# mkkellogg/GaussianSplats3D

Measured on AMD Instinct MI355X. Metric: Msplats/s sorted+rasterized at 1920x1080 SH-2, higher is better.
Workload: dtype int32 keys / f32 raster; 1 GPU; C3: garden.ply stand-in, SH2, 1920x1080; splats=5800000, sh_degree=2, width=1920, height=1080, cull=off (R=N), sort_precision_bits=16, streams=one (SURVEY.md 8d: sort -> draw on a single stream), parallelism=1 GPU, sort=full list (R = N)

## Files before the change

### gaussiansplats3d_amd/csrc/extreme_set.cpp

```cpp
#include "extreme_set.hpp"

#include <math.h>

#include <algorithm>
#include <new>
#include <utility>

namespace {

typedef __int128 i128;

struct P { int32_t x, y, z; };
inline bool operator==(const P& a, const P& b) { return a.x == b.x && a.y == b.y && a.z == b.z; }
inline bool lex_less(const P& a, const P& b) { return a.x != b.x ? a.x < b.x : (a.y != b.y ? a.y < b.y : a.z < b.z); }
struct D3 { int64_t x, y, z; };
inline D3 sub(const P& a, const P& b) { return {(int64_t)a.x - b.x, (int64_t)a.y - b.y, (int64_t)a.z - b.z}; }
struct N3 { i128 x, y, z; };
inline N3 cross(const D3& u, const D3& v) {
    return {(i128)u.y * v.z - (i128)u.z * v.y, (i128)u.z * v.x - (i128)u.x * v.z, (i128)u.x * v.y - (i128)u.y * v.x};
}
inline i128 dot(const N3& n, const D3& d) { return n.x * d.x + n.y * d.y + n.z * d.z; }
inline bool is_zero(const N3& n) { return n.x == 0 && n.y == 0 && n.z == 0; }
inline double len2(const N3& n) { return (double)n.x * (double)n.x + (double)n.y * (double)n.y + (double)n.z * (double)n.z; }
inline double dabs128(i128 v) { return fabs((double)v); }
// ... 266 lines not shown
        } else {
            if (h.vert.size() > cap || flt.work > budget) break;
            if (round >= 1 && now > (size_t)64 * cap && now * 10 > prev * 7) break;
            if (round >= 2 && now * 100 > prev * 97) break;
        }
        prev = now;
        size_t joined = 0;
        for (size_t f = 0; f < flt.best.size(); f++)
            if (flt.best[f] > 0 && h.insert(flt.best_p[f])) joined++;
        if (!joined) break;
    }
    if (s.size() > cap) return false;
    dedupe(s);
    out.swap(s);
    return true;
}

}

bool gs_extreme_set(const int32_t* a, size_t na, const int32_t* b, size_t nb, uint32_t cap, std::vector<int32_t>& out) {
    out.clear();
    try {
        std::vector<P> s;
        const Src src = {a, na, b, nb};
        if (!build(src, cap, s)) return false;
        emit(s, out);
        return true;
    } catch (const std::bad_alloc&) {
        out.clear();
        return false;
    }
}

extern "C" int gs_debug_extreme_set(const int32_t* prior_aos4, uint32_t prior_count, const int32_t* aos4, uint32_t count, uint32_t cap,
                                    int32_t* out_aos4, uint32_t* out_count) {
    if (!out_aos4 || !out_count || (prior_count && !prior_aos4) || (count && !aos4)) return -1;
    *out_count = 0;
    std::vector<int32_t> out;
    if (!gs_extreme_set(prior_aos4, prior_count, aos4, count, cap, out)) return 1;
    std::copy(out.begin(), out.end(), out_aos4);
    *out_count = (uint32_t)(out.size() / 4);
    return 0;
}
```

### gaussiansplats3d_amd/csrc/extreme_set.hpp

```cpp
#pragma once
#include <cstddef>
#include <cstdint>
#include <vector>

constexpr uint32_t GS_EXTREME_CAP = 4096;

bool gs_extreme_set(const int32_t* a, size_t na, const int32_t* b, size_t nb, uint32_t cap, std::vector<int32_t>& out);

extern "C" int gs_debug_extreme_set(const int32_t* prior_aos4, uint32_t prior_count, const int32_t* aos4, uint32_t count, uint32_t cap,
                                    int32_t* out_aos4, uint32_t* out_count);
```

### gaussiansplats3d_amd/csrc/gs_internal.hpp

```cpp
#pragma once
#include <hip/hip_runtime.h>
#include <stdint.h>
#include <stdio.h>
#include <stdlib.h>
#include <string.h>
#include <new>
#include <utility>
#include <vector>

#include "../../include/gsplat_hip.h"
#include "draw_plan.hpp"

void gs_set_error(const char* fmt, ...);

#define GS_HIP(expr)                                                                              \
    do {                                                                                          \
        hipError_t _e = (expr);                                                                   \
        if (_e != hipSuccess) {                                                                   \
            gs_set_error("%s failed: %s (%s:%d)", #expr, hipGetErrorString(_e), __FILE__, __LINE__); \
            return GS_ERR_HIP;                                                                    \
        }                                                                                         \
    } while (0)

#define GS_REQUIRE(cond, msg)                                    \
// ... 210 lines not shown
    gs_mesh* result_mesh = nullptr;
    const uint32_t* result_unmap = nullptr;
    uint32_t result_payload_max = 0;
    uint32_t gathered = 0;
    bool has_gathered = false;
    bool gathered_on_device = false;
    DevBuf gathered_dev;
    gs_tree* pending_tree = nullptr;
    bool pending_keep_zeroed = false;
    uint32_t centers_version = 0;
    DevBuf pay_in;
    DevBuf leaf_centers, leaf_pos;
    uint64_t leaf_cache_tree = 0;
    uint32_t leaf_cache_centers = 0, leaf_cache_layout = 0, leaf_cache_uploaded = 0;
    const void* leaf_cache_mesh = nullptr;
    uint32_t last_render = 0, last_sort = 0, last_passes = 0;
    bool last_identity = true;
    bool has_result = false;
    bool frustum_cull = false;
    bool visibility_cull = false;
    bool last_culled = false;
    const SortFrame* result_frame = nullptr;
    DevBuf keep_mask;
    DevBuf chunk_counts;
    DevBuf mask_copy;
    bool last_vis_culled = false;
    bool dev_distances = false;
    uint32_t dev_distances_count = 0;
    bool dev_distances_integer = false;
    hipEvent_t ev_handover = nullptr;
    std::vector<int32_t> extreme;
    bool extreme_ok = true;
    uint32_t extreme_version = 0;
    uint32_t clean_slot = 3;
    bool last_known_range = false;
    int32_t last_range_lo = 0, last_range_hi = 0;
    uint32_t last_pass0_slot = 0;
    bool last_narrow = false;
    bool keys_stale = false;
    int32_t stale_im[3] = {0, 0, 0};
    uint32_t stale_count = 0;
};

struct __attribute__((aligned(32))) SplatRec {
    float cx, cy, ax, ay;
    float bx, by;
    uint32_t c0, c1;
};
static_assert(sizeof(SplatRec) == 32, "SplatRec must be one 32-byte sector");

struct RenderFrame {
    uint32_t visible;
    uint32_t entries_lo;
    uint32_t entries_hi;
    uint32_t overflow;
    uint32_t entry_count;
    uint32_t tiles16_lo;
    uint32_t tiles16_hi;
    uint32_t pad;
};

struct ProjectParams {
    float view[16];
    float proj[16];
    float cam_pos[3];
    float focal_x, focal_y;
    float width, height;
    float splat_scale, kernel2d, max_splat_px, inv_focal_adj;
    uint32_t sh_degree;
    uint32_t sh_stored;
    uint32_t cov_half;
// ... 173 lines not shown
```

### gaussiansplats3d_amd/csrc/sorter.hip

```cpp
#include <math.h>
#include <stdlib.h>

#include "extreme_set.hpp"
#include "radix.hpp"

__host__ __device__ static inline int32_t trunc_f64_i32(double v) {
    if (!(v > -2147483649.0 && v < 2147483648.0)) return INT32_MIN;
    return (int32_t)v;
}

constexpr uint32_t MODE_INT = 1, MODE_DYNAMIC = 2, MODE_PRECOMPUTED = 4;
#ifndef GS_KEY_GRID_MULT
#define GS_KEY_GRID_MULT 2
#endif

struct SceneRows {
    int32_t im[GS_MAX_SCENES][4];
    float fm[GS_MAX_SCENES][4];
};

struct KeyParams {
    const uint32_t *cx, *cy, *cz, *cw;
    const uint4* aos;
    const uint32_t* scene_idx;
// ... 2 lines not shown
    const SceneRows* rows;
    int32_t* keys_out;
    SortFrame* frame;
    SortFrame* next_frame;
    uint32_t* digit_total;
    uint32_t sort_start, render_count, mode;
    uint32_t last_splat;
    int32_t im0, im1, im2;
    float fm0, fm1, fm2;
    float mvp[16];
    unsigned long long* keep;
    const uint32_t* count_dev;
    uint32_t ext_minmax;
};

__global__ __launch_bounds__(256) void k_store_scene_rows(SceneRows rows, SceneRows* __restrict__ dst) {
    const uint32_t t = threadIdx.x;
    if (t < GS_MAX_SCENES * 4) {
        dst->im[t >> 2][t & 3] = rows.im[t >> 2][t & 3];
        dst->fm[t >> 2][t & 3] = rows.fm[t >> 2][t & 3];
    }
}

__global__ __launch_bounds__(256) void k_aos4_to_soa(const uint4* __restrict__ aos, uint32_t count, uint32_t from,
                                                     uint32_t* __restrict__ x, uint32_t* __restrict__ y,
                                                     uint32_t* __restrict__ z, uint32_t* __restrict__ w) {
    for (uint32_t i = blockIdx.x * blockDim.x + threadIdx.x; i < count; i += gridDim.x * blockDim.x) {
        const uint4 v = aos[i];
        x[from + i] = v.x;
        y[from + i] = v.y;
        z[from + i] = v.z;
        if (w) w[from + i] = v.w;
    }
}

__device__ __forceinline__ int32_t static_key_int(const KeyParams& p, uint32_t x, uint32_t y, uint32_t z) {
    return (int32_t)(x * (uint32_t)p.im0 + y * (uint32_t)p.im1 + z * (uint32_t)p.im2);
}
__device__ __forceinline__ int32_t static_key_float(const KeyParams& p, uint32_t xb, uint32_t yb, uint32_t zb) {
    float s = __fmul_rn(p.fm0, __uint_as_float(xb));
    s = __fadd_rn(s, __fmul_rn(p.fm1, __uint_as_float(yb)));
    s = __fadd_rn(s, __fmul_rn(p.fm2, __uint_as_float(zb)));
    return trunc_f64_i32((double)s * 4096.0);
}
__device__ __forceinline__ int32_t static_key(const KeyParams& p, uint32_t x, uint32_t y, uint32_t z) {
    return (p.mode & MODE_INT) ? static_key_int(p, x, y, z) : static_key_float(p, x, y, z);
}
__device__ __forceinline__ int32_t static_key_planes(const KeyParams& p, uint32_t i) {
    if (p.mode & MODE_INT) return static_key_int(p, p.cx[i], p.cy[i], p.cz[i]);
    return static_key_float(p, p.cx[i], p.cy[i], p.cz[i]);
}
__device__ __forceinline__ int4 static_key_int4(const KeyParams& p, const uint4& x, const uint4& y, const uint4& z) {
    return make_int4(static_key_int(p, x.x, y.x, z.x), static_key_int(p, x.y, y.y, z.y), static_key_int(p, x.z, y.z, z.z),
                     static_key_int(p, x.w, y.w, z.w));
}

__device__ __forceinline__ float3 centre_int_as_float(uint32_t x, uint32_t y, uint32_t z) {
    return make_float3(__fmul_rn((float)(int32_t)x, 0.001f), __fmul_rn((float)(int32_t)y, 0.001f), __fmul_rn((float)(int32_t)z, 0.001f));
}
__device__ __forceinline__ int32_t static_key_centre(const KeyParams& p, const uint4& c, float3& centre) {
    if (p.mode & MODE_INT) {
        centre = centre_int_as_float(c.x, c.y, c.z);
        return static_key_int(p, c.x, c.y, c.z);
    }
    centre = make_float3(__uint_as_float(c.x), __uint_as_float(c.y), __uint_as_float(c.z));
    return static_key_float(p, c.x, c.y, c.z);
// ... 679 lines not shown
    const uint32_t* __restrict__ words;
    const uint32_t* __restrict__ n_dev;
    uint32_t n_host, val_bits;
    __device__ __forceinline__ void prepare() {}
    __device__ __forceinline__ uint32_t count() const { return n_dev ? *n_dev : n_host; }
    struct Raw { uint32_t w; };
    __device__ __forceinline__ uint32_t pre(uint32_t) const { return 0u; }
    __device__ __forceinline__ Raw fetch(uint32_t j, uint32_t) const { return Raw{ld32(words, j)}; }
    __device__ __forceinline__ void decode(const Raw& r, uint32_t& k, uint32_t& v) const {
        k = r.w >> val_bits;
        v = r.w & ((1u << val_bits) - 1u);
    }
    __device__ __forceinline__ bool valid(uint32_t) const { return true; }
    static __device__ __forceinline__ int prof_slot(int) { return 1; }
};

__global__ void k_copy_head(const uint32_t* __restrict__ idx, const uint32_t* __restrict__ map, uint32_t* __restrict__ out,
                            uint32_t n, uint32_t last_splat) {
    for (uint32_t i = blockIdx.x * blockDim.x + threadIdx.x; i < n; i += gridDim.x * blockDim.x) {
        const uint32_t o = idx ? min(idx[i], last_splat) : i;
        out[i] = map ? map[o] : o;
    }
}

__global__ void k_unmap(const uint32_t* __restrict__ in, const uint32_t* __restrict__ unmap, uint32_t* __restrict__ out,
                        uint32_t n, uint32_t last) {
    for (uint32_t i = blockIdx.x * blockDim.x + threadIdx.x; i < n; i += gridDim.x * blockDim.x) out[i] = unmap[min(in[i], last)];
}

constexpr uint32_t KEY_HIST_VECS = 3;
#ifndef GS_KEY_HIST_PAIR
#define GS_KEY_HIST_PAIR 1
#endif
template <bool NARROW>
__global__ __launch_bounds__(HIST_THREADS) void k_depth_key_hist(KeyParams p, DepthLoader ld, int32_t key_lo, int32_t key_hi, int shift,
                                                                  uint32_t keep_slot, uint32_t* __restrict__ block_hist,
                                                                  uint32_t* __restrict__ group_rows, uint16_t* __restrict__ keys16) {
    __shared__ uint32_t s_hist[4][RADIX_BINS];
    const uint32_t tid = threadIdx.x, t = blockIdx.x * HIST_THREADS + tid;
    sort_begin(p, t, gridDim.x * HIST_THREADS, keep_slot);
    if (t < SORT_SHARDS) {
        p.frame->key_min[t] = key_lo;
        p.frame->key_max[t] = key_hi;
    }
    ld.set_known_range(key_lo, key_hi);
    for (uint32_t k = tid; k < 4u * RADIX_BINS; k += HIST_THREADS) (&s_hist[0][0])[k] = 0;
    __syncthreads();
    uint32_t* hist = s_hist[(tid >> 6) & 3u];
    const uint32_t R = p.render_count;
    const RadixChunk ch = radix_chunk(R);
    const uint32_t j0 = min(ch.tile_begin * (uint32_t)RADIX_TILE, R), j1 = min(ch.tile_end * (uint32_t)RADIX_TILE, R);
    const uint32_t p0 = R - j1, p1 = R - j0;
    auto count = [&](int32_t k) {
        const uint32_t r = ld.hist_key(k);
        atomicAdd(&hist[(r >> shift) & 255u], 1u);
        return r;
    };
    auto scalars = [&](uint32_t begin, uint32_t end) {
        for (uint32_t i = begin + tid; i < end; i += HIST_THREADS) {
            const int32_t k = static_key_int(p, p.cx[i], p.cy[i], p.cz[i]);
            const uint32_t r = count(k);
            if (NARROW) keys16[i] = (uint16_t)r;
            else p.keys_out[i] = k;
        }
    };
    constexpr uint32_t VPU = (NARROW && GS_KEY_HIST_PAIR) ? 2u : 1u, UPOS = 4u * VPU;
    constexpr uint32_t UNITS = VPU == 2u ? (uint32_t)(GS_KEY_HIST_PAIR ? GS_KEY_HIST_PAIR : 1) : KEY_HIST_VECS;
    const uint32_t a = (p0 + UPOS - 1u) / UPOS, b = p1 / UPOS;
    if (a < b) {
        scalars(p0, a * UPOS);
        scalars(b * UPOS, p1);
        const uint4* x4 = reinterpret_cast<const uint4*>(p.cx);
        const uint4* y4 = reinterpret_cast<const uint4*>(p.cy);
        const uint4* z4 = reinterpret_cast<const uint4*>(p.cz);
        int4* o4 = reinterpret_cast<int4*>(p.keys_out);
        for (uint32_t u0 = a; u0 < b; u0 += UNITS * HIST_THREADS) {
            uint4 x[UNITS][VPU], y[UNITS][VPU], z[UNITS][VPU];
#pragma unroll
            for (uint32_t k = 0; k < UNITS; k++) {
                const uint32_t u = min(u0 + k * HIST_THREADS + tid, b - 1u);
#pragma unroll
                for (uint32_t q = 0; q < VPU; q++) { x[k][q] = x4[u * VPU + q]; y[k][q] = y4[u * VPU + q]; z[k][q] = z4[u * VPU + q]; }
            }
#pragma unroll
            for (uint32_t k = 0; k < UNITS; k++) {
                const uint32_t u = u0 + k * HIST_THREADS + tid;
                int4 key[VPU];
#pragma unroll
                for (uint32_t q = 0; q < VPU; q++) key[q] = static_key_int4(p, x[k][q], y[k][q], z[k][q]);
                if (u < b) {
                    if constexpr (NARROW) {
                        uint32_t w[2u * VPU];
#pragma unroll
                        for (uint32_t q = 0; q < VPU; q++) {
                            const uint32_t r0 = count(key[q].x), r1 = count(key[q].y), r2 = count(key[q].z), r3 = count(key[q].w);
                            w[2u * q] = r0 | (r1 << 16);
                            w[2u * q + 1u] = r2 | (r3 << 16);
                        }
                        if constexpr (VPU == 2u) reinterpret_cast<uint4*>(keys16)[u] = make_uint4(w[0], w[1], w[2], w[3]);
                        else reinterpret_cast<uint2*>(keys16)[u] = make_uint2(w[0], w[1]);
                    } else {
                        o4[u] = key[0];
                        count(key[0].x); count(key[0].y); count(key[0].z); count(key[0].w);
                    }
                }
            }
        }
    } else {
        scalars(p0, p1);
    }
    __syncthreads();
    if (tid >= RADIX_BINS || ch.tile_begin >= ch.tile_end) return;
    const uint32_t total = s_hist[0][tid] + s_hist[1][tid] + s_hist[2][tid] + s_hist[3][tid];
    block_hist[ch.id * RADIX_BINS + tid] = total;
    if (total) atomicAdd(&group_rows[(ch.id / RADIX_GROUP) * RADIX_BINS + tid], total);
}

__global__ void k_debug_buckets(DepthLoader ld, int32_t* out) {
    ld.prepare();
    for (uint32_t i = ld.sort_start + blockIdx.x * blockDim.x + threadIdx.x; i < ld.render_count;
         i += gridDim.x * blockDim.x)
        out[i] = (int32_t)ld.bucket(i);
}

__global__ __launch_bounds__(256) void k_debug_rekey(KeyParams p, uint32_t n) {
    for (uint32_t i = blockIdx.x * blockDim.x + threadIdx.x; i < n; i += gridDim.x * blockDim.x)
        p.keys_out[i] = static_key_int(p, p.cx[i], p.cy[i], p.cz[i]);
}

struct Pass0Args {
    DepthLoaderArgs ld;
    uint32_t Rs, val_bits;
    int shift;
    bool pack, chunked, wide;
    void* kbuf0;
    uint32_t* vo;
// ... 108 lines not shown
    static const bool off = getenv("GSPLAT_NO_KNOWN_RANGE") != nullptr;
    return off;
}

static int sorter_update_extreme(gs_sorter* s, uint32_t from, uint32_t end, uint32_t old_uploaded, bool zero_fill) {
    if (s->flags != GS_SORT_INTEGER || known_range_off()) return GS_OK;
    const bool current = s->extreme_ok && s->extreme_version + 1u == s->centers_version;
    const bool append = from >= old_uploaded;
    if (append && !current) {
        s->extreme_ok = false;
        return GS_OK;
    }
    const uint32_t first = append ? old_uploaded : 0u, last = end > old_uploaded ? end : old_uploaded;
    std::vector<int32_t> rows, out;
    try {
        if (zero_fill && append) rows.assign(4, 0);
        else rows.resize((size_t)(last - first) * 4);
    } catch (const std::bad_alloc&) {
        s->extreme_ok = false;
        return GS_OK;
    }
    if (!(zero_fill && append) && last > first) {
        GS_HIP(hipMemcpyAsync(rows.data(), s->caos.as<uint4>() + first, (size_t)(last - first) * 16, hipMemcpyDeviceToHost, s->stream));
        GS_HIP(hipStreamSynchronize(s->stream));
    }
    const bool prior = append && !s->extreme.empty();
    s->extreme_ok = gs_extreme_set(prior ? s->extreme.data() : nullptr, prior ? s->extreme.size() / 4 : 0, rows.data(), rows.size() / 4,
                                   GS_EXTREME_CAP, out);
    s->extreme.swap(out);
    s->extreme_version = s->centers_version;
    return GS_OK;
}

static int sorter_refresh_keys(gs_sorter* s) {
    if (!s->keys_stale) return GS_OK;
    KeyParams kp = {};
    kp.cx = s->cx.as<uint32_t>(); kp.cy = s->cy.as<uint32_t>(); kp.cz = s->cz.as<uint32_t>();
    kp.keys_out = s->keys.as<int32_t>();
    kp.mode = MODE_INT;
    kp.im0 = s->stale_im[0]; kp.im1 = s->stale_im[1]; kp.im2 = s->stale_im[2];
    hipLaunchKernelGGL(k_debug_rekey, dim3(grid_for(s->stale_count, 1024, 2048)), dim3(256), 0, s->stream, kp, s->stale_count);
    GS_HIP(hipGetLastError());
    s->keys_stale = false;
    return GS_OK;
}

int gs_sorter_upload_centers(gs_sorter* s, uint32_t from, uint32_t count, const void* centers_aos4,
                             const uint32_t* scene_indexes) {
    GS_REQUIRE(s && centers_aos4, "sorter / centers == NULL");
    GS_REQUIRE((uint64_t)from + count <= s->max_count, "range exceeds max_splat_count");
    GS_REQUIRE(!(s->flags & GS_SORT_DYNAMIC) || scene_indexes, "dynamic sorter needs scene_indexes");
    if (count == 0) return GS_OK;
    ScopedDevice sd(s->ctx->device);
    GS_TRY(sorter_refresh_keys(s));
    GS_HIP(hipMemcpyAsync(s->caos.as<uint4>() + from, centers_aos4, (size_t)count * 16, hipMemcpyHostToDevice, s->stream));
    return gs_sorter_commit_centers(s, from, count, scene_indexes);
}

}

int gs_sorter_commit_centers(gs_sorter* s, uint32_t from, uint32_t count, const uint32_t* scene_indexes) {
    hipStream_t st = s->stream;
    GS_TRY(sorter_refresh_keys(s));
    uint4* aos = s->caos.as<uint4>() + from;
    hipLaunchKernelGGL(k_aos4_to_soa, dim3(grid_for(count, 256, 4096)), dim3(256), 0, st, aos, count,
                       from, s->cx.as<uint32_t>(), s->cy.as<uint32_t>(), s->cz.as<uint32_t>(),
                       (s->flags & GS_SORT_DYNAMIC) ? s->cw.as<uint32_t>() : nullptr);
    GS_HIP(hipGetLastError());
    if (s->flags & GS_SORT_DYNAMIC)
        GS_HIP(hipMemcpyAsync(s->scene_idx.as<uint32_t>() + from, scene_indexes, (size_t)count * 4, hipMemcpyHostToDevice, st));
    GS_HIP(hipStreamSynchronize(st));
    const uint32_t old_uploaded = s->uploaded;
    if (from + count > s->uploaded) s->uploaded = from + count;
    s->centers_version++;
    GS_TRY(sorter_update_extreme(s, from, from + count, old_uploaded, false));
    sorter_tell_mesh(s);
    return GS_OK;
}

extern "C" {

int gs_sorter_set_uploaded_count(gs_sorter* s, uint32_t count) {
    GS_REQUIRE(s != nullptr, "sorter == NULL");
    GS_REQUIRE(count <= s->max_count, "count exceeds max_splat_count");
    if (count <= s->uploaded) return GS_OK;
    ScopedDevice sd(s->ctx->device);
    hipStream_t st = s->stream;
    const size_t from = s->uploaded, n = count - s->uploaded;
    GS_HIP(hipMemsetAsync(s->caos.as<uint4>() + from, 0, n * 16, st));
    DevBuf* planes[] = {&s->cx, &s->cy, &s->cz, &s->cw, &s->scene_idx};
    for (DevBuf* b : planes)
        if (b->p) GS_HIP(hipMemsetAsync(b->as<uint32_t>() + from, 0, n * 4, st));
    GS_HIP(hipStreamSynchronize(st));
    s->uploaded = count;
    s->centers_version++;
    GS_TRY(sorter_update_extreme(s, (uint32_t)from, count, (uint32_t)from, true));
    sorter_tell_mesh(s);
    return GS_OK;
}

static int sorter_collect_stats(gs_sorter* s, gs_sort_stats* stats) {
    SortFrame f;
    GS_HIP(hipMemcpyAsync(&f, s->frame.as<SortFrame>() + s->frame_index, sizeof(f), hipMemcpyDeviceToHost, s->stream));
    GS_HIP(hipStreamSynchronize(s->stream));
    float ms = 0.f;
    if (s->timed_sort) GS_HIP(hipEventElapsedTime(&ms, s->ev0, s->ev1));
    int32_t key_lo = f.lo(), key_hi = f.hi();
    if (s->last_sort == 0) {
        key_lo = KEY_MIN_INIT;
        key_hi = KEY_MAX_INIT;
        f.clamped = 0;
    }
    stats->device_ms = ms;
    stats->key_min = key_lo;
    stats->key_max = key_hi;
    stats->clamped = f.clamped;
    stats->passes = s->last_passes;
    stats->result_count = s->last_culled ? f.kept : s->last_render;
    return f.clamped ? GS_WARN_KEY_CLAMPED : GS_OK;
}

struct SortSwitches {
    bool tree_no_fuse;
    const char* vis_front;
    bool no_pack;
    bool no_chunk;
    bool no_known_range;
    bool no_narrow_keys;
};
static SortSwitches sort_switches() {
    static const bool tree_no_fuse = getenv("GSPLAT_TREE_NO_FUSE") != nullptr;
    static const char* vis_front = getenv("GSPLAT_VIS_FRONT");
    static const bool no_pack = getenv("GSPLAT_NO_SORT_PACK") != nullptr;
    static const bool no_chunk = getenv("GSPLAT_NO_SORT_CHUNK") != nullptr;
    static const bool no_narrow_keys = getenv("GSPLAT_NO_NARROW_KEYS") != nullptr;
    return {tree_no_fuse, vis_front, no_pack, no_chunk, known_range_off(), no_narrow_keys};
}

static bool sorter_mesh_alive(const gs_context* ctx, const gs_mesh* m) {
    for (const gs_mesh* l : ctx->live_meshes)
        if (l == m) return m != nullptr;
    return false;
}

struct ChunkGrid { uint32_t grid, len; };
static ChunkGrid chunk_grid(const gs_context* ctx, uint32_t R, uint32_t unit) {
    const uint32_t units = (R + unit - 1u) / unit;
    const uint32_t grid = units < (uint32_t)ctx->cu_count * 2u ? units : (uint32_t)ctx->cu_count * 2u;
    return {grid, ((units + grid - 1u) / grid) * unit};
}

struct SortPlan {
    const float* mvp;
    const uint32_t* indexes_to_sort;
    bool device_list;
    const void* precomputed;
    const float* transforms;
    const uint32_t* list_count_dev;
    uint32_t R, Rs, sort_start;
    bool pre_device, dynamic;
    bool vis_cull;
    bool cull;
    const uint32_t *map, *unmap;
    uint32_t last_splat;
    uint32_t max_payload, val_bits;
    SortSwitches sw;
    const uint32_t* idx_dev;
    bool fused_tree;
    bool vec4;
    bool vis_front;
    bool known_range;
    int32_t range_lo, range_hi;
    bool narrow;
    uint32_t pass0_slot;
};

struct Pass0Shape { bool pack, chunked; uint32_t grid; };
static Pass0Shape pass0_shape(const gs_sorter* s, const SortPlan& pl) {
    Pass0Shape sh;
    sh.chunked = !pl.sw.no_chunk && pl.val_bits <= 24u && radix_chunk_grid_for(pl.Rs) != 0u;
    sh.pack = s->precision > 8u && !pl.sw.no_pack && (s->precision - 8u) + pl.val_bits <= 32u;
    sh.grid = (sh.pack && sh.chunked) ? radix_chunk_grid_for(pl.Rs) : radix_grid_for(pl.Rs);
    return sh;
}

static bool sort_known_range(const gs_sorter* s, const SortPlan& pl, const KeyParams& kp, int32_t& lo_out, int32_t& hi_out) {
    if (pl.sw.no_known_range || kp.mode != MODE_INT || pl.idx_dev || pl.device_list || pl.fused_tree || pl.vis_cull || pl.cull ||
        pl.list_count_dev || pl.sort_start != 0u || pl.R != s->uploaded || pl.R == 0u)
        return false;
    if (!s->extreme_ok || s->extreme_version != s->centers_version || s->extreme.empty()) return false;
    const int32_t* c = s->extreme.data();
    const size_t n = s->extreme.size() / 4;
    const int64_t a0 = kp.im0, a1 = kp.im1, a2 = kp.im2;
    const int64_t small = (int64_t)1 << 29;
    __int128 lo, hi;
    if (a0 >= -small && a0 <= small && a1 >= -small && a1 <= small && a2 >= -small && a2 <= small) {
        int64_t l = INT64_MAX, h = INT64_MIN;
        for (size_t i = 0; i < n; i++) {
            const int64_t v = a0 * c[4 * i] + a1 * c[4 * i + 1] + a2 * c[4 * i + 2];
            l = v < l ? v : l;
            h = v > h ? v : h;
        }
        lo = l; hi = h;
    } else {
        lo = hi = (__int128)a0 * c[0] + (__int128)a1 * c[1] + (__int128)a2 * c[2];
        for (size_t i = 1; i < n; i++) {
// ... 200 lines not shown
        else hipLaunchKernelGGL(k_mask_count, dim3(wg.grid), dim3(VC_THREADS), 0, st, kp, mask, wg.len, counts);
        if (pl.map) hipLaunchKernelGGL(k_cull_front<true>, dim3(wg.grid), dim3(VC_THREADS), 0, st, kp, mask, s->mask_copy.as<uint32_t>(),
                                       counts, wg.len, pl.map, s->pay_in.as<uint32_t>(), lazy ? DERIVE_SUBS : 1u);
        else hipLaunchKernelGGL(k_cull_front<false>, dim3(wg.grid), dim3(VC_THREADS), 0, st, kp, mask, s->mask_copy.as<uint32_t>(),
                                counts, wg.len, pl.map, s->pay_in.as<uint32_t>(), 1u);
    } else {
        const ChunkGrid cg = chunk_grid(ctx, R, VC_SPAN);
        if (!s->pending_tree) s->has_gathered = false;
        GS_TRY(s->chunk_counts.ensure((size_t)std::max(lazy ? dg.grid * DERIVE_SUBS : 0u, cg.grid) * 4));
        counts = s->chunk_counts.as<uint32_t>();
        if (lazy) derive();
        hipLaunchKernelGGL(k_minmax_count, dim3(cg.grid), dim3(VC_THREADS), 0, st, kp, mask, cg.len, counts);
        hipLaunchKernelGGL(k_mask_compact, dim3(cg.grid), dim3(VC_THREADS), 0, st, mask, s->mask_copy.as<uint32_t>(), counts, R, cg.len,
                           s->idx_in.as<uint32_t>(), kp.frame);
    }
    if (R >= mesh->vis_orig_count && (!lazy || mesh->vis_orig_tail_zero)) mesh->vis_orig_dirty = false;
    pl.idx_dev = s->idx_in.as<uint32_t>();
    kp.idx_in = pl.idx_dev;
    kp.count_dev = &kp.frame->kept;
    kp.ext_minmax = 1u;
    if (!pl.vis_front) hipLaunchKernelGGL(k_depth_key<false>, dim3(grid_for(pl.Rs, 256 * 4, (uint32_t)ctx->cu_count * 2)), dim3(256), 0, st, kp);
    return GS_OK;
}

static int launch_front_end(gs_sorter* s, SortPlan& pl, KeyParams& kp) {
    gs_context* ctx = s->ctx;
    hipStream_t st = s->stream;
    const uint32_t cus = (uint32_t)ctx->cu_count;
    pl.vec4 = (kp.mode == MODE_INT) && !pl.idx_dev;
    pl.known_range = sort_known_range(s, pl, kp, pl.range_lo, pl.range_hi);
    pl.pass0_slot = pl.known_range ? s->clean_slot : 0u;
    s->clean_slot = pl.pass0_slot == 3u ? 0u : 3u;
    pl.narrow = pl.known_range && s->precision <= 16u && !pl.sw.no_narrow_keys;
    if (pl.known_range) {
        DepthLoaderArgs hl = {};
        hl.keys = s->keys.as<int32_t>(); hl.frame = kp.frame; hl.sort_start = 0u; hl.render_count = pl.R; hl.range = 1u << s->precision;
        hl.last_splat = kp.last_splat; hl.count_clamps = 1u;
        const dim3 grid(pass0_shape(s, pl).grid);
        uint32_t* group_rows = s->radix.digit_total.as<uint32_t>() + pl.pass0_slot * RADIX_SLOT_WORDS;
        if (pl.narrow)
            hipLaunchKernelGGL(k_depth_key_hist<true>, grid, dim3(HIST_THREADS), 0, st, kp, DepthLoader{hl}, pl.range_lo, pl.range_hi, 0,
                               pl.pass0_slot, s->radix.block_hist.as<uint32_t>(), group_rows, s->keys16.as<uint16_t>());
        else
            hipLaunchKernelGGL(k_depth_key_hist<false>, grid, dim3(HIST_THREADS), 0, st, kp, DepthLoader{hl}, pl.range_lo, pl.range_hi, 0,
                               pl.pass0_slot, s->radix.block_hist.as<uint32_t>(), group_rows, (uint16_t*)nullptr);
    } else if (pl.fused_tree) {
        GS_TRY(launch_tree_front(s, pl, kp));
    } else if (pl.vis_cull) {
        GS_TRY(launch_vis_cull_front(s, pl, kp));
    } else if (pl.cull) {
        if (pl.vec4) hipLaunchKernelGGL(k_depth_key_cull<true>, dim3(grid_for(pl.Rs, 256 * 16, cus * 2)), dim3(256), 0, st, kp);
        else hipLaunchKernelGGL(k_depth_key_cull<false>, dim3(grid_for(pl.Rs, 256 * 4, cus * 4)), dim3(256), 0, st, kp);
    } else if (pl.vec4) {
        hipLaunchKernelGGL(k_depth_key<true>, dim3(grid_for(pl.Rs, 256 * 16, cus * GS_KEY_GRID_MULT)), dim3(256), 0, st, kp);
    } else {
        hipLaunchKernelGGL(k_depth_key<false>, dim3(grid_for(pl.Rs, 256 * 4, cus * 2)), dim3(256), 0, st, kp);
    }
    GS_HIP(hipGetLastError());
    return GS_OK;
}

static int run_radix_passes(gs_sorter* s, const SortPlan& pl, const KeyParams& kp) {
    const RadixExec ex = {s->stream, &s->radix, s->ctx->lds_atomic_lane_order};
    const uint32_t Rs = pl.Rs, val_bits = pl.val_bits;
    const bool own_payloads = pl.fused_tree || pl.vis_front;
    DepthLoaderArgs dl = {};
    dl.keys = s->keys.as<int32_t>();
    dl.keys16 = s->keys16.as<uint16_t>();
    dl.keep = pl.cull ? kp.keep : nullptr;
    dl.idx = own_payloads ? s->pay_in.as<uint32_t>() : pl.idx_dev;
    dl.map = own_payloads ? nullptr : pl.map;
    dl.frame = kp.frame;
    dl.sort_start = pl.sort_start;
    dl.render_count = pl.R;
    dl.range = 1u << s->precision;
    dl.last_splat = own_payloads ? pl.max_payload : kp.last_splat;
    dl.n_dev = pl.vis_cull ? &kp.frame->kept : pl.list_count_dev;
    const uint32_t passes = (s->precision + 7) / 8;
// ... 31 lines not shown
            else if (last) GS_TRY((radix_pass_ex<ArrayLoader<uint32_t>, PackedLoader, uint8_t, false, false, false>(ex, ph, (int)val_bits, pk, Rs, 0, (int)p, (uint8_t*)nullptr, vo, nullptr, 0u, 0u)));
            else GS_TRY((radix_pass_ex<ArrayLoader<uint32_t>, PackedLoader, uint8_t, false, false, true>(ex, ph, (int)val_bits, pk, Rs, 0, (int)p, (uint8_t*)nullptr, vo, nullptr, 0u, val_bits)));
        } else if (wide) {
            ArrayLoader<uint32_t> al = {(const uint32_t*)kbuf[(p - 1) & 1], vbuf[(p - 1) & 1], n_dev, Rs};
            if (last) GS_TRY((radix_pass<ArrayLoader<uint32_t>, uint32_t, false>(ex, al, al, Rs, shift, (int)p, (uint32_t*)nullptr, vo)));
            else if (pack) GS_TRY((radix_pass_ex<ArrayLoader<uint32_t>, ArrayLoader<uint32_t>, uint8_t, false, false, true>(ex, al, shift, al, Rs, shift, (int)p, (uint8_t*)nullptr, vo, nullptr, 0u, val_bits)));
            else GS_TRY((radix_pass<ArrayLoader<uint32_t>, uint32_t, true>(ex, al, al, Rs, shift, (int)p, (uint32_t*)kbuf[p & 1], vo)));
        } else {
            ArrayLoader<uint16_t> al = {(const uint16_t*)kbuf[(p - 1) & 1], vbuf[(p - 1) & 1], n_dev, Rs};
            if (last) GS_TRY((radix_pass<ArrayLoader<uint16_t>, uint16_t, false>(ex, al, al, Rs, shift, (int)p, (uint16_t*)nullptr, vo)));
            else GS_TRY((radix_pass<ArrayLoader<uint16_t>, uint16_t, true>(ex, al, al, Rs, shift, (int)p, (uint16_t*)kbuf[p & 1], vo)));
        }
        in_packed = in_packed || pack;
    }
    return GS_OK;
}

static int sort_finish(gs_sorter* s, const SortPlan& pl, const KeyParams& kp, uint32_t passes, uint32_t* sorted_out, gs_sort_stats* stats) {
    hipStream_t st = s->stream;
    if (pl.sort_start > 0) {
        hipLaunchKernelGGL(k_copy_head, dim3(grid_for(pl.sort_start, 1024, 2048)), dim3(256), 0, st, pl.idx_dev, pl.map,
                           s->sorted.as<uint32_t>(), pl.sort_start, s->uploaded - 1u);
    }
    GS_HIP(hipGetLastError());
    if (s->timed_sort || st != s->ctx->stream) GS_HIP(hipEventRecord(s->ev1, st));
    s->last_render = pl.R;
    s->last_sort = pl.Rs;
    s->last_passes = passes;
    s->last_known_range = pl.known_range;
    s->last_range_lo = pl.known_range ? pl.range_lo : 0;
    s->last_range_hi = pl.known_range ? pl.range_hi : 0;
    s->last_pass0_slot = pl.pass0_slot;
    s->last_narrow = pl.narrow;
    if (pl.Rs > 0) {
        s->keys_stale = pl.narrow;
        s->stale_im[0] = kp.im0; s->stale_im[1] = kp.im1; s->stale_im[2] = kp.im2;
        s->stale_count = pl.R;
    }
    s->last_identity = (pl.idx_dev == nullptr);
    s->last_culled = (pl.cull || pl.vis_cull || pl.list_count_dev) && pl.Rs > 0;
    s->last_vis_culled = pl.vis_cull && pl.Rs > 0;
    s->result_frame = kp.frame;
    s->result_mesh = pl.map ? s->bound_mesh : nullptr;
    s->result_unmap = pl.unmap;
    s->result_payload_max = pl.max_payload;
    s->has_result = true;

    uint32_t out_count = pl.R;
    if (sorted_out && s->last_culled) {
        SortFrame f;
        GS_HIP(hipMemcpyAsync(&f, kp.frame, sizeof(f), hipMemcpyDeviceToHost, st));
        GS_HIP(hipStreamSynchronize(st));
        out_count = f.kept;
    }
    if (sorted_out && out_count) {
        const void* src = s->sorted.p;
        if (pl.unmap) {
            GS_TRY(s->debug.ensure((size_t)s->max_count * 4));
            hipLaunchKernelGGL(k_unmap, dim3(grid_for(out_count, 1024, 2048)), dim3(256), 0, st, s->sorted.as<uint32_t>(), pl.unmap,
                               s->debug.as<uint32_t>(), out_count, s->result_payload_max);
            GS_HIP(hipGetLastError());
            src = s->debug.p;
        }
        GS_HIP(hipMemcpyAsync(sorted_out, src, (size_t)out_count * 4, hipMemcpyDeviceToHost, st));
        GS_HIP(hipStreamSynchronize(st));
    }
// ... 54 lines not shown
    if (s->bound_mesh != m && sorter_mesh_alive(s->ctx, s->bound_mesh)) s->bound_mesh->derive_orig_mask = false;
    s->bound_mesh = m;
    sorter_tell_mesh(s);
    return GS_OK;
}

int gs_sorter_set_frustum_cull(gs_sorter* s, int enable) {
    GS_REQUIRE(s != nullptr, "sorter == NULL");
    GS_REQUIRE(!enable || !(s->flags & GS_SORT_DYNAMIC), "the per-splat frustum cull is not available to a dynamic-mode sorter");
    s->frustum_cull = enable != 0;
    return GS_OK;
}

int gs_sorter_set_visibility_cull(gs_sorter* s, int enable) {
    GS_REQUIRE(s != nullptr, "sorter == NULL");
    GS_REQUIRE(!enable || !(s->flags & GS_SORT_DYNAMIC), "the visibility cull is not available to a dynamic-mode sorter");
    s->visibility_cull = enable != 0;
    sorter_tell_mesh(s);
    return GS_OK;
}

int gs_sorter_last_stats(gs_sorter* s, gs_sort_stats* stats) {
    GS_REQUIRE(s && stats, "sorter / stats == NULL");
    GS_REQUIRE(s->has_result, "no sort has run");
    ScopedDevice sd(s->ctx->device);
    return sorter_collect_stats(s, stats);
}

int gs_sorter_debug_read(gs_sorter* s, int what, void* dst, uint32_t count) {
    GS_REQUIRE(s && dst, "sorter / dst == NULL");
    GS_REQUIRE(s->has_result, "no sort has run");
    if (what == 4) {
        const bool valid = s->extreme_ok && s->extreme_version == s->centers_version;
        const int32_t w[7] = {s->last_known_range ? 1 : 0, valid ? (int32_t)(s->extreme.size() / 4) : 0, s->last_range_lo, s->last_range_hi,
                              valid ? 1 : 0, (int32_t)s->last_pass0_slot, s->last_narrow ? 1 : 0};
        GS_REQUIRE(count <= 7u, "selector 4 holds 7 words");
        memcpy(dst, w, (size_t)count * 4);
        return GS_OK;
    }
    GS_REQUIRE(count <= s->last_render, "count exceeds the last render_count");
    ScopedDevice sd(s->ctx->device);
    hipStream_t st = s->stream;
    const void* src = nullptr;
    if (what == 0 || what == 1) GS_TRY(sorter_refresh_keys(s));
    if (what == 0) src = s->keys.p;
    else if (what == 2) {
        src = s->sorted.p;
        if (sorter_mesh_alive(s->ctx, s->result_mesh) && s->result_unmap && count) {
            GS_TRY(s->debug.ensure((size_t)s->max_count * 4));
            hipLaunchKernelGGL(k_unmap, dim3(grid_for(count, 1024, 2048)), dim3(256), 0, st, s->sorted.as<uint32_t>(),
                               s->result_unmap, s->debug.as<uint32_t>(), count, s->result_payload_max);
            GS_HIP(hipGetLastError());
            src = s->debug.p;
        }
    }
    else if (what == 1) {
        GS_TRY(s->debug.ensure((size_t)s->max_count * 4));
        DepthLoaderArgs dl = {};
        dl.keys = s->keys.as<int32_t>();
        dl.frame = s->frame.as<SortFrame>() + s->frame_index;
        dl.sort_start = s->last_render - s->last_sort;
        dl.render_count = s->last_render;
        dl.range = 1u << s->precision;
        GS_HIP(hipMemsetAsync(s->debug.p, 0, (size_t)s->last_render * 4, st));
        if (s->last_sort)
            hipLaunchKernelGGL(k_debug_buckets, dim3(grid_for(s->last_sort, 1024, 2048)), dim3(256), 0, st, DepthLoader{dl}, s->debug.as<int32_t>());
        GS_HIP(hipGetLastError());
        src = s->debug.p;
    } else if (what == 3) {
// ... 18 lines not shown
```

Measured before the change: 25760 Msplats/s.

## Store 16-bit offset centre planes for narrow-key histogram pass

```diff
diff --git a/gaussiansplats3d_amd/csrc/extreme_set.cpp b/gaussiansplats3d_amd/csrc/extreme_set.cpp
--- a/gaussiansplats3d_amd/csrc/extreme_set.cpp
+++ b/gaussiansplats3d_amd/csrc/extreme_set.cpp
@@ -322,6 +322,27 @@
     }
 }
 
+bool gs_compact_offsets(const int32_t* set_aos4, size_t n, int32_t offset[3]) {
+    if (!set_aos4 || n == 0) return false;
+    int32_t lo[3], hi[3];
+    for (int k = 0; k < 3; k++) lo[k] = hi[k] = set_aos4[k];
+    for (size_t i = 1; i < n; i++)
+        for (int k = 0; k < 3; k++) {
+            const int32_t v = set_aos4[4 * i + k];
+            lo[k] = std::min(lo[k], v);
+            hi[k] = std::max(hi[k], v);
+        }
+    for (int k = 0; k < 3; k++)
+        if ((int64_t)hi[k] - (int64_t)lo[k] > 65535) return false;
+    for (int k = 0; k < 3; k++) offset[k] = lo[k];
+    return true;
+}
+
+extern "C" int gs_debug_compact_offsets(const int32_t* set_aos4, uint32_t count, int32_t* offset3) {
+    if (!offset3 || (count && !set_aos4)) return -1;
+    return gs_compact_offsets(set_aos4, count, offset3) ? 1 : 0;
+}
+
 extern "C" int gs_debug_extreme_set(const int32_t* prior_aos4, uint32_t prior_count, const int32_t* aos4, uint32_t count, uint32_t cap,
                                     int32_t* out_aos4, uint32_t* out_count) {
     if (!out_aos4 || !out_count || (prior_count && !prior_aos4) || (count && !aos4)) return -1;
diff --git a/gaussiansplats3d_amd/csrc/extreme_set.hpp b/gaussiansplats3d_amd/csrc/extreme_set.hpp
--- a/gaussiansplats3d_amd/csrc/extreme_set.hpp
+++ b/gaussiansplats3d_amd/csrc/extreme_set.hpp
@@ -7,5 +7,9 @@
 
 bool gs_extreme_set(const int32_t* a, size_t na, const int32_t* b, size_t nb, uint32_t cap, std::vector<int32_t>& out);
 
+bool gs_compact_offsets(const int32_t* set_aos4, size_t n, int32_t offset[3]);
+
+extern "C" int gs_debug_compact_offsets(const int32_t* set_aos4, uint32_t count, int32_t* offset3);
+
 extern "C" int gs_debug_extreme_set(const int32_t* prior_aos4, uint32_t prior_count, const int32_t* aos4, uint32_t count, uint32_t cap,
                                     int32_t* out_aos4, uint32_t* out_count);
diff --git a/gaussiansplats3d_amd/csrc/gs_internal.hpp b/gaussiansplats3d_amd/csrc/gs_internal.hpp
--- a/gaussiansplats3d_amd/csrc/gs_internal.hpp
+++ b/gaussiansplats3d_amd/csrc/gs_internal.hpp
@@ -266,11 +266,17 @@
     std::vector<int32_t> extreme;
     bool extreme_ok = true;
     uint32_t extreme_version = 0;
+    DevBuf cx16, cy16, cz16;
+    DevBuf c16_bad;
+    bool c16_ok = false;
+    uint32_t c16_version = 0;
+    int32_t c16_off[3] = {0, 0, 0};
     uint32_t clean_slot = 3;
     bool last_known_range = false;
     int32_t last_range_lo = 0, last_range_hi = 0;
     uint32_t last_pass0_slot = 0;
     bool last_narrow = false;
+    bool last_compact = false;
     bool keys_stale = false;
     int32_t stale_im[3] = {0, 0, 0};
     uint32_t stale_count = 0;
diff --git a/gaussiansplats3d_amd/csrc/sorter.hip b/gaussiansplats3d_amd/csrc/sorter.hip
--- a/gaussiansplats3d_amd/csrc/sorter.hip
+++ b/gaussiansplats3d_amd/csrc/sorter.hip
@@ -58,6 +58,21 @@
         z[from + i] = v.z;
         if (w) w[from + i] = v.w;
     }
+}
+
+__global__ __launch_bounds__(256) void k_compact_centres(const int32_t* __restrict__ x, const int32_t* __restrict__ y,
+                                                         const int32_t* __restrict__ z, uint32_t from, uint32_t end, int32_t ox, int32_t oy,
+                                                         int32_t oz, uint16_t* __restrict__ x16, uint16_t* __restrict__ y16,
+                                                         uint16_t* __restrict__ z16, uint32_t* __restrict__ bad) {
+    uint32_t nbad = 0;
+    for (uint32_t i = from + blockIdx.x * blockDim.x + threadIdx.x; i < end; i += gridDim.x * blockDim.x) {
+        const int64_t dx = (int64_t)x[i] - ox, dy = (int64_t)y[i] - oy, dz = (int64_t)z[i] - oz;
+        nbad += (dx < 0 || dx > 65535 || dy < 0 || dy > 65535 || dz < 0 || dz > 65535) ? 1u : 0u;
+        x16[i] = (uint16_t)dx;
+        y16[i] = (uint16_t)dy;
+        z16[i] = (uint16_t)dz;
+    }
+    if (nbad) atomicAdd(bad, nbad);
 }
 
 __device__ __forceinline__ int32_t static_key_int(const KeyParams& p, uint32_t x, uint32_t y, uint32_t z) {
@@ -803,10 +818,22 @@
 #ifndef GS_KEY_HIST_PAIR
 #define GS_KEY_HIST_PAIR 1
 #endif
-template <bool NARROW>
+#ifndef GS_KEY_HIST_C16_UNITS
+#define GS_KEY_HIST_C16_UNITS 1
+#endif
+struct CompactCentres {
+    const uint16_t *x, *y, *z;
+    uint32_t k0;
+};
+__device__ __forceinline__ int32_t compact_key_int(const KeyParams& p, uint32_t k0, uint32_t dx, uint32_t dy, uint32_t dz) {
+    return (int32_t)(k0 + dx * (uint32_t)p.im0 + dy * (uint32_t)p.im1 + dz * (uint32_t)p.im2);
+}
+template <bool NARROW, bool COMPACT = false>
 __global__ __launch_bounds__(HIST_THREADS) void k_depth_key_hist(KeyParams p, DepthLoader ld, int32_t key_lo, int32_t key_hi, int shift,
                                                                   uint32_t keep_slot, uint32_t* __restrict__ block_hist,
-                                                                  uint32_t* __restrict__ group_rows, uint16_t* __restrict__ keys16) {
+                                                                  uint32_t* __restrict__ group_rows, uint16_t* __restrict__ keys16,
+                                                                  CompactCentres cc) {
+    static_assert(NARROW || !COMPACT, "the 16-bit centre planes feed the 16-bit radix keys only");
     __shared__ uint32_t s_hist[4][RADIX_BINS];
     const uint32_t tid = threadIdx.x, t = blockIdx.x * HIST_THREADS + tid;
     sort_begin(p, t, gridDim.x * HIST_THREADS, keep_slot);
@@ -829,50 +856,77 @@
     };
     auto scalars = [&](uint32_t begin, uint32_t end) {
         for (uint32_t i = begin + tid; i < end; i += HIST_THREADS) {
-            const int32_t k = static_key_int(p, p.cx[i], p.cy[i], p.cz[i]);
+            const int32_t k = COMPACT ? compact_key_int(p, cc.k0, cc.x[i], cc.y[i], cc.z[i]) : static_key_int(p, p.cx[i], p.cy[i], p.cz[i]);
             const uint32_t r = count(k);
             if (NARROW) keys16[i] = (uint16_t)r;
             else p.keys_out[i] = k;
         }
     };
-    constexpr uint32_t VPU = (NARROW && GS_KEY_HIST_PAIR) ? 2u : 1u, UPOS = 4u * VPU;
+    constexpr uint32_t VPU = (NARROW && GS_KEY_HIST_PAIR) ? 2u : 1u, UPOS = COMPACT ? 8u : 4u * VPU;
     constexpr uint32_t UNITS = VPU == 2u ? (uint32_t)(GS_KEY_HIST_PAIR ? GS_KEY_HIST_PAIR : 1) : KEY_HIST_VECS;
     const uint32_t a = (p0 + UPOS - 1u) / UPOS, b = p1 / UPOS;
     if (a < b) {
         scalars(p0, a * UPOS);
         scalars(b * UPOS, p1);
-        const uint4* x4 = reinterpret_cast<const uint4*>(p.cx);
-        const uint4* y4 = reinterpret_cast<const uint4*>(p.cy);
-        const uint4* z4 = reinterpret_cast<const uint4*>(p.cz);
-        int4* o4 = reinterpret_cast<int4*>(p.keys_out);
-        for (uint32_t u0 = a; u0 < b; u0 += UNITS * HIST_THREADS) {
-            uint4 x[UNITS][VPU], y[UNITS][VPU], z[UNITS][VPU];
-#pragma unroll
-            for (uint32_t k = 0; k < UNITS; k++) {
-                const uint32_t u = min(u0 + k * HIST_THREADS + tid, b - 1u);
-#pragma unroll
-                for (uint32_t q = 0; q < VPU; q++) { x[k][q] = x4[u * VPU + q]; y[k][q] = y4[u * VPU + q]; z[k][q] = z4[u * VPU + q]; }
+        if constexpr (COMPACT) {
+            constexpr uint32_t CU = GS_KEY_HIST_C16_UNITS;
+            const uint4* x8 = reinterpret_cast<const uint4*>(cc.x);
+            const uint4* y8 = reinterpret_cast<const uint4*>(cc.y);
+            const uint4* z8 = reinterpret_cast<const uint4*>(cc.z);
+            auto two = [&](uint32_t xw, uint32_t yw, uint32_t zw) {
+                const uint32_t r0 = count(compact_key_int(p, cc.k0, xw & 0xFFFFu, yw & 0xFFFFu, zw & 0xFFFFu));
+                const uint32_t r1 = count(compact_key_int(p, cc.k0, xw >> 16, yw >> 16, zw >> 16));
+                return r0 | (r1 << 16);
+            };
+            for (uint32_t u0 = a; u0 < b; u0 += CU * HIST_THREADS) {
+                uint4 x[CU], y[CU], z[CU];
+#pragma unroll
+                for (uint32_t k = 0; k < CU; k++) {
+                    const uint32_t u = min(u0 + k * HIST_THREADS + tid, b - 1u);
+                    x[k] = x8[u]; y[k] = y8[u]; z[k] = z8[u];
+                }
+#pragma unroll
+                for (uint32_t k = 0; k < CU; k++) {
+                    const uint32_t u = u0 + k * HIST_THREADS + tid;
+                    if (u < b)
+                        reinterpret_cast<uint4*>(keys16)[u] = make_uint4(two(x[k].x, y[k].x, z[k].x), two(x[k].y, y[k].y, z[k].y),
+                                                                         two(x[k].z, y[k].z, z[k].z), two(x[k].w, y[k].w, z[k].w));
+                }
             }
-#pragma unroll
-            for (uint32_t k = 0; k < UNITS; k++) {
-                const uint32_t u = u0 + k * HIST_THREADS + tid;
-                int4 key[VPU];
-#pragma unroll
-                for (uint32_t q = 0; q < VPU; q++) key[q] = static_key_int4(p, x[k][q], y[k][q], z[k][q]);
-                if (u < b) {
-                    if constexpr (NARROW) {
-                        uint32_t w[2u * VPU];
-#pragma unroll
-                        for (uint32_t q = 0; q < VPU; q++) {
-                            const uint32_t r0 = count(key[q].x), r1 = count(key[q].y), r2 = count(key[q].z), r3 = count(key[q].w);
-                            w[2u * q] = r0 | (r1 << 16);
-                            w[2u * q + 1u] = r2 | (r3 << 16);
+        } else {
+            const uint4* x4 = reinterpret_cast<const uint4*>(p.cx);
+            const uint4* y4 = reinterpret_cast<const uint4*>(p.cy);
+            const uint4* z4 = reinterpret_cast<const uint4*>(p.cz);
+            int4* o4 = reinterpret_cast<int4*>(p.keys_out);
+            for (uint32_t u0 = a; u0 < b; u0 += UNITS * HIST_THREADS) {
+                uint4 x[UNITS][VPU], y[UNITS][VPU], z[UNITS][VPU];
+#pragma unroll
+                for (uint32_t k = 0; k < UNITS; k++) {
+                    const uint32_t u = min(u0 + k * HIST_THREADS + tid, b - 1u);
+#pragma unroll
+                    for (uint32_t q = 0; q < VPU; q++) { x[k][q] = x4[u * VPU + q]; y[k][q] = y4[u * VPU + q]; z[k][q] = z4[u * VPU + q]; }
+                }
+#pragma unroll
+                for (uint32_t k = 0; k < UNITS; k++) {
+                    const uint32_t u = u0 + k * HIST_THREADS + tid;
+                    int4 key[VPU];
+#pragma unroll
+                    for (uint32_t q = 0; q < VPU; q++) key[q] = static_key_int4(p, x[k][q], y[k][q], z[k][q]);
+                    if (u < b) {
+                        if constexpr (NARROW) {
+                            uint32_t w[2u * VPU];
+#pragma unroll
+                            for (uint32_t q = 0; q < VPU; q++) {
+                                const uint32_t r0 = count(key[q].x), r1 = count(key[q].y), r2 = count(key[q].z), r3 = count(key[q].w);
+                                w[2u * q] = r0 | (r1 << 16);
+                                w[2u * q + 1u] = r2 | (r3 << 16);
+                            }
+                            if constexpr (VPU == 2u) reinterpret_cast<uint4*>(keys16)[u] = make_uint4(w[0], w[1], w[2], w[3]);
+                            else reinterpret_cast<uint2*>(keys16)[u] = make_uint2(w[0], w[1]);
+                        } else {
+                            o4[u] = key[0];
+                            count(key[0].x); count(key[0].y); count(key[0].z); count(key[0].w);
                         }
-                        if constexpr (VPU == 2u) reinterpret_cast<uint4*>(keys16)[u] = make_uint4(w[0], w[1], w[2], w[3]);
-                        else reinterpret_cast<uint2*>(keys16)[u] = make_uint2(w[0], w[1]);
-                    } else {
-                        o4[u] = key[0];
-                        count(key[0].x); count(key[0].y); count(key[0].z); count(key[0].w);
                     }
                 }
             }
@@ -1047,6 +1101,41 @@
     return GS_OK;
 }
 
+static bool compact_centres_off() {
+    static const bool off = getenv("GSPLAT_NO_COMPACT_CENTRES") != nullptr;
+    return off;
+}
+
+static int sorter_update_compact(gs_sorter* s, uint32_t from, uint32_t end, uint32_t old_uploaded) {
+    const bool was_current = s->c16_ok && s->c16_version + 1u == s->centers_version;
+    s->c16_ok = false;
+    if (s->flags != GS_SORT_INTEGER || compact_centres_off() || s->uploaded == 0u) return GS_OK;
+    if (!s->extreme_ok || s->extreme_version != s->centers_version) return GS_OK;
+    int32_t off[3];
+    if (!gs_compact_offsets(s->extreme.data(), s->extreme.size() / 4, off)) return GS_OK;
+    const size_t bytes = (size_t)s->max_count * 2 + 16;
+    bool fresh[3];
+    GS_TRY(s->cx16.ensure(bytes, &fresh[0])); GS_TRY(s->cy16.ensure(bytes, &fresh[1])); GS_TRY(s->cz16.ensure(bytes, &fresh[2]));
+    GS_TRY(s->c16_bad.ensure(4));
+    const bool keep = was_current && !fresh[0] && !fresh[1] && !fresh[2] && off[0] == s->c16_off[0] && off[1] == s->c16_off[1] &&
+                      off[2] == s->c16_off[2];
+    from = keep ? std::min(from, old_uploaded) : 0u;
+    if (!keep) end = s->uploaded;
+    hipStream_t st = s->stream;
+    uint32_t bad = 1u;
+    GS_HIP(hipMemsetAsync(s->c16_bad.p, 0, 4, st));
+    hipLaunchKernelGGL(k_compact_centres, dim3(grid_for(end - from, 1024, 4096)), dim3(256), 0, st, s->cx.as<int32_t>(), s->cy.as<int32_t>(),
+                       s->cz.as<int32_t>(), from, end, off[0], off[1], off[2], s->cx16.as<uint16_t>(), s->cy16.as<uint16_t>(),
+                       s->cz16.as<uint16_t>(), s->c16_bad.as<uint32_t>());
+    GS_HIP(hipGetLastError());
+    GS_HIP(hipMemcpyAsync(&bad, s->c16_bad.p, 4, hipMemcpyDeviceToHost, st));
+    GS_HIP(hipStreamSynchronize(st));
+    memcpy(s->c16_off, off, sizeof(off));
+    s->c16_version = s->centers_version;
+    s->c16_ok = bad == 0u;
+    return GS_OK;
+}
+
 static int sorter_refresh_keys(gs_sorter* s) {
     if (!s->keys_stale) return GS_OK;
     KeyParams kp = {};
@@ -1089,6 +1178,7 @@
     if (from + count > s->uploaded) s->uploaded = from + count;
     s->centers_version++;
     GS_TRY(sorter_update_extreme(s, from, from + count, old_uploaded, false));
+    GS_TRY(sorter_update_compact(s, from, from + count, old_uploaded));
     sorter_tell_mesh(s);
     return GS_OK;
 }
@@ -1110,6 +1200,7 @@
     s->uploaded = count;
     s->centers_version++;
     GS_TRY(sorter_update_extreme(s, (uint32_t)from, count, (uint32_t)from, true));
+    GS_TRY(sorter_update_compact(s, (uint32_t)from, count, (uint32_t)from));
     sorter_tell_mesh(s);
     return GS_OK;
 }
@@ -1142,6 +1233,7 @@
     bool no_chunk;
     bool no_known_range;
     bool no_narrow_keys;
+    bool no_compact_centres;
 };
 static SortSwitches sort_switches() {
     static const bool tree_no_fuse = getenv("GSPLAT_TREE_NO_FUSE") != nullptr;
@@ -1149,7 +1241,7 @@
     static const bool no_pack = getenv("GSPLAT_NO_SORT_PACK") != nullptr;
     static const bool no_chunk = getenv("GSPLAT_NO_SORT_CHUNK") != nullptr;
     static const bool no_narrow_keys = getenv("GSPLAT_NO_NARROW_KEYS") != nullptr;
-    return {tree_no_fuse, vis_front, no_pack, no_chunk, known_range_off(), no_narrow_keys};
+    return {tree_no_fuse, vis_front, no_pack, no_chunk, known_range_off(), no_narrow_keys, compact_centres_off()};
 }
 
 static bool sorter_mesh_alive(const gs_context* ctx, const gs_mesh* m) {
@@ -1187,6 +1279,7 @@
     bool known_range;
     int32_t range_lo, range_hi;
     bool narrow;
+    bool compact;
     uint32_t pass0_slot;
 };
 
@@ -1453,18 +1546,27 @@
     pl.pass0_slot = pl.known_range ? s->clean_slot : 0u;
     s->clean_slot = pl.pass0_slot == 3u ? 0u : 3u;
     pl.narrow = pl.known_range && s->precision <= 16u && !pl.sw.no_narrow_keys;
+    pl.compact = pl.narrow && !pl.sw.no_compact_centres && s->c16_ok && s->c16_version == s->centers_version;
     if (pl.known_range) {
         DepthLoaderArgs hl = {};
         hl.keys = s->keys.as<int32_t>(); hl.frame = kp.frame; hl.sort_start = 0u; hl.render_count = pl.R; hl.range = 1u << s->precision;
         hl.last_splat = kp.last_splat; hl.count_clamps = 1u;
         const dim3 grid(pass0_shape(s, pl).grid);
         uint32_t* group_rows = s->radix.digit_total.as<uint32_t>() + pl.pass0_slot * RADIX_SLOT_WORDS;
-        if (pl.narrow)
+        CompactCentres cc = {};
+        if (pl.compact) {
+            cc.x = s->cx16.as<uint16_t>(); cc.y = s->cy16.as<uint16_t>(); cc.z = s->cz16.as<uint16_t>();
+            cc.k0 = (uint32_t)s->c16_off[0] * (uint32_t)kp.im0 + (uint32_t)s->c16_off[1] * (uint32_t)kp.im1 +
+                    (uint32_t)s->c16_off[2] * (uint32_t)kp.im2;
+            hipLaunchKernelGGL((k_depth_key_hist<true, true>), grid, dim3(HIST_THREADS), 0, st, kp, DepthLoader{hl}, pl.range_lo, pl.range_hi,
+                               0, pl.pass0_slot, s->radix.block_hist.as<uint32_t>(), group_rows, s->keys16.as<uint16_t>(), cc);
+        } else if (pl.narrow) {
             hipLaunchKernelGGL(k_depth_key_hist<true>, grid, dim3(HIST_THREADS), 0, st, kp, DepthLoader{hl}, pl.range_lo, pl.range_hi, 0,
-                               pl.pass0_slot, s->radix.block_hist.as<uint32_t>(), group_rows, s->keys16.as<uint16_t>());
-        else
+                               pl.pass0_slot, s->radix.block_hist.as<uint32_t>(), group_rows, s->keys16.as<uint16_t>(), cc);
+        } else {
             hipLaunchKernelGGL(k_depth_key_hist<false>, grid, dim3(HIST_THREADS), 0, st, kp, DepthLoader{hl}, pl.range_lo, pl.range_hi, 0,
-                               pl.pass0_slot, s->radix.block_hist.as<uint32_t>(), group_rows, (uint16_t*)nullptr);
+                               pl.pass0_slot, s->radix.block_hist.as<uint32_t>(), group_rows, (uint16_t*)nullptr, cc);
+        }
     } else if (pl.fused_tree) {
         GS_TRY(launch_tree_front(s, pl, kp));
     } else if (pl.vis_cull) {
@@ -1562,6 +1664,7 @@
     s->last_range_hi = pl.known_range ? pl.range_hi : 0;
     s->last_pass0_slot = pl.pass0_slot;
     s->last_narrow = pl.narrow;
+    s->last_compact = pl.compact;
     if (pl.Rs > 0) {
         s->keys_stale = pl.narrow;
         s->stale_im[0] = kp.im0; s->stale_im[1] = kp.im1; s->stale_im[2] = kp.im2;
@@ -1682,9 +1785,9 @@
     GS_REQUIRE(s->has_result, "no sort has run");
     if (what == 4) {
         const bool valid = s->extreme_ok && s->extreme_version == s->centers_version;
-        const int32_t w[7] = {s->last_known_range ? 1 : 0, valid ? (int32_t)(s->extreme.size() / 4) : 0, s->last_range_lo, s->last_range_hi,
-                              valid ? 1 : 0, (int32_t)s->last_pass0_slot, s->last_narrow ? 1 : 0};
-        GS_REQUIRE(count <= 7u, "selector 4 holds 7 words");
+        const int32_t w[8] = {s->last_known_range ? 1 : 0, valid ? (int32_t)(s->extreme.size() / 4) : 0, s->last_range_lo, s->last_range_hi,
+                              valid ? 1 : 0, (int32_t)s->last_pass0_slot, s->last_narrow ? 1 : 0, s->last_compact ? 1 : 0};
+        GS_REQUIRE(count <= 8u, "selector 4 holds 8 words");
         memcpy(dst, w, (size_t)count * 4);
         return GS_OK;
     }
```

Measured after the change: 26670 Msplats/s (median of 6 runs). 1.04x the previous value.
